# vsahni3/cross-attention-ViT

Hardware: AMD Instinct MI355X
Metric: 3D patch-tokens/sec fwd+bwd, 2-modality 128^3 p16 ViT (higher is better)
Workload: dtype bf16; 1 GPU; configs[1]: ModelCross d=768 H=12 mlp=3072 2x2 blocks, 2 modalities, 128^3 volume, 16^3 patches (N=513), dropout 0; per_gpu_batch=126, global_batch=126, seq_len=513, parallelism=dp1, step=zero-grad + weight bf16 cast + fwd + loss + bwd, optimizer_step=excluded, launch=eager (one launch per kernel)

## Files before the change

cross-attention-vit_amd/csrc/gemm.hip:

```cpp
#include "xvit_common.h"

#include <atomic>
#include <algorithm>
#include <string>

namespace xvit {

struct GemmParams {
  const bf16* A = nullptr; const bf16* B = nullptr; void* C = nullptr; const float* bias = nullptr; const float* res = nullptr; bf16* aux = nullptr;
  int64_t lda = 0, ldb = 0, ldc = 0, ldr = 0, ldaux = 0;
  int64_t sA = 0, sB = 0, sC = 0, sBias = 0, sR = 0, sAux = 0;
  int M = 0, N = 0, K = 0, k_per_split = 0, split_k = 1, ntm = 0, ntn = 0;
  int c_f32 = 0, act = XVIT_ACT_NONE, accumulate = 0;
  int res_row_mod = 0, res_row_off = 0, seg_rows = 0, seg_skip = 0, row_off = 0;
  float* slab = nullptr;
  float* colsum = nullptr;
  float drop_p = 0.f, drop_inv = 1.f; uint64_t drop_seed = 0;
  const uint64_t* drop_epoch = nullptr;
  int aux_deriv = 0;
  int narrow_epi = 0;
  int ncg = 1;
  int res_in_body = 0;
  struct PatchGather {
    int mode = 0;
    int dp, hp, wp;
    int Dn, Wn;
    int Sy, Sz;
    int pcount, ntok, cls;
    int nb;
    int64_t sBt, sMd;
    uint32_t vol_bytes;
    uint32_t m_pcount, m_dn, m_wn, m_nb;
    uint32_t m_ntok;
  } g;
};

constexpr uint32_t GATHER_OOB = 0x80000000u;
constexpr uint32_t OOB = 0xFFFFFFF0u;
typedef __attribute__((__vector_size__(2 * sizeof(unsigned)))) unsigned u32x2_t;
typedef __attribute__((__vector_size__(4 * sizeof(unsigned)))) unsigned u32x4_t;
__device__ __forceinline__ uint32_t gather_elem_off(const GemmParams::PatchGather& g, int e) {
  const int hw = g.hp * g.wp, p1 = e / hw, r = e - p1 * hw, p2 = r / g.wp, p3 = r - p2 * g.wp;
  return (uint32_t)(p1 * g.Sz + p2 * g.Sy + p3);
}
__device__ __forceinline__ uint32_t gather_patch_origin(const GemmParams::PatchGather& g, int q) {
  const int d = q % g.Dn, t = q / g.Dn, w = t % g.Wn, h = t / g.Wn;
  return (uint32_t)(d * g.dp * g.Sz + h * g.hp * g.Sy + w * g.wp);
}
__device__ __forceinline__ uint32_t gather_sample_origin(const GemmParams::PatchGather& g, int s) {
  const int mod = s / g.nb, b = s - mod * g.nb;
  return (uint32_t)(b * g.sBt + mod * g.sMd);
}

__device__ __forceinline__ uint32_t fast_div(uint32_t n, uint32_t d, uint32_t m, uint32_t& rem) {
  uint32_t q = __umulhi(n, m);
  rem = n - q * d;
  if (rem >= d) { ++q; rem -= d; }
  return q;
}
struct GatherTok { uint32_t row, vol; bool ok; };
__device__ __forceinline__ GatherTok gather_token(const GemmParams::PatchGather& g, uint32_t T, uint32_t total) {
  GatherTok o;
  o.ok = T < total;
  uint32_t q, b, d, w;
  const uint32_t smp = fast_div(o.ok ? T : 0u, (uint32_t)g.pcount, g.m_pcount, q);
  const uint32_t mod = fast_div(smp, (uint32_t)g.nb, g.m_nb, b);
  const uint32_t t = fast_div(q, (uint32_t)g.Dn, g.m_dn, d);
  const uint32_t h = fast_div(t, (uint32_t)g.Wn, g.m_wn, w);
  o.row = smp * (uint32_t)g.ntok + (uint32_t)g.cls + q;
  o.vol = (uint32_t)(b * g.sBt + mod * g.sMd) + d * (uint32_t)(g.dp * g.Sz) + h * (uint32_t)(g.hp * g.Sy) + w * (uint32_t)g.wp;
  return o;
}

constexpr int ACT_GELU_D = 3;
constexpr int ACT_MULAUX = 4;

template <int ACT>
__device__ __forceinline__ void act4(f32x4& v, f32x4& d, const bf16x4 z) {
  if (ACT == XVIT_ACT_GELU || ACT == ACT_GELU_D) {
#pragma unroll
    for (int c = 0; c < 4; ++c) { float a_, d_; gelu_and_grad(v[c], a_, d_); v[c] = a_; d[c] = d_; }
  } else if (ACT == XVIT_ACT_DGELU) {
#pragma unroll
    for (int c = 0; c < 4; ++c) v[c] *= dgelu_f(bf2f(z[c]));
  } else if (ACT == ACT_MULAUX) {
#pragma unroll
    for (int c = 0; c < 4; ++c) v[c] *= bf2f(z[c]);
  }
}
__device__ __forceinline__ void dropout4(const GemmParams& p, f32x4& v, uint64_t idx) {
  const uint32_t thr = (uint32_t)(p.drop_p * kTwo24);
  const uint64_t seed = drop_seed_at(p.drop_seed, p.drop_epoch);
#pragma unroll
  for (int c = 0; c < 4; ++c) v[c] = draw24(seed, idx + c) >= thr ? v[c] * p.drop_inv : 0.f;
}
template <int GROUP>
__device__ __forceinline__ void colsum_flush(float* dst, f32x4 cs, bool col_ok) {
#pragma unroll
  for (int c = 0; c < 4; ++c) {
    float t = cs[c];
#pragma unroll
    for (int o = GROUP; o < 64; o <<= 1) t += __shfl_xor(t, o);
    cs[c] = t;
  }
  if ((threadIdx.x & 63) < GROUP && col_ok) {
#pragma unroll
    for (int c = 0; c < 4; ++c) unsafeAtomicAdd(dst + c, cs[c]);
  }
}

template <int ACT, bool DROP = false>
__device__ __forceinline__ f32x4 epilogue_apply(const GemmParams& p, f32x4 v, int row, int col, int64_t cb, const float* bias, const float* res,
                                                bf16* aux) {
  if (bias) v += *(const f32x4*)(bias + col);
  if (ACT == XVIT_ACT_GELU) {
    f32x4 d;
    const f32x4 zv = v;
    act4<XVIT_ACT_GELU>(v, d, bf16x4{});
    if (aux) {
      const f32x4 s = p.aux_deriv ? d : zv;
      *(bf16x4*)(aux + (int64_t)row * p.ldaux + col) = to_bf16x4(s);
    }
  } else if (ACT == XVIT_ACT_DGELU) {
    const bf16x4 z = *(const bf16x4*)(aux + (int64_t)row * p.ldaux + col);
    f32x4 d;
    if (p.aux_deriv) act4<ACT_MULAUX>(v, d, z);
    else act4<XVIT_ACT_DGELU>(v, d, z);
  }
  if (DROP) dropout4(p, v, (uint64_t)(cb / (p.sC ? p.sC : 1)) * ((uint64_t)p.M * p.N) + (uint64_t)row * p.N + col);
  if (res) {
    const int rr = p.res_row_mod > 0 ? p.res_row_off + (row % p.res_row_mod) : row;
    v += *(const f32x4*)(res + (int64_t)rr * p.ldr + col);
  }
  const int64_t orow = p.seg_rows > 0 ? (int64_t)row + (row / p.seg_rows) * p.seg_skip + p.row_off : row;
  if (p.c_f32) {
    float* dst = (float*)p.C + cb + orow * p.ldc + col;
    if (p.accumulate) v += *(const f32x4*)dst;
    *(f32x4*)dst = v;
  } else {
    *(bf16x4*)((bf16*)p.C + cb + orow * p.ldc + col) = to_bf16x4(v);
  }
  return v;
}
__device__ __forceinline__ f32x4 epilogue_apply_rt(const GemmParams& p, f32x4 v, int row, int col, int64_t cb, const float* bias, const float* res,
                                                   bf16* aux) {
  if (p.drop_p > 0.f) {
    if (p.act == XVIT_ACT_GELU) return epilogue_apply<XVIT_ACT_GELU, true>(p, v, row, col, cb, bias, res, aux);
    if (p.act == XVIT_ACT_DGELU) return epilogue_apply<XVIT_ACT_DGELU, true>(p, v, row, col, cb, bias, res, aux);
    return epilogue_apply<XVIT_ACT_NONE, true>(p, v, row, col, cb, bias, res, aux);
  }
  if (p.act == XVIT_ACT_GELU) return epilogue_apply<XVIT_ACT_GELU>(p, v, row, col, cb, bias, res, aux);
  if (p.act == XVIT_ACT_DGELU) return epilogue_apply<XVIT_ACT_DGELU>(p, v, row, col, cb, bias, res, aux);
  return epilogue_apply<XVIT_ACT_NONE>(p, v, row, col, cb, bias, res, aux);
}

constexpr int BM = 128, BN = 128, BK = 64;
constexpr int OPER_BYTES = BM * BK * 2;
constexpr int STAGE_BYTES = 2 * OPER_BYTES;
// ... 556 lines not shown
  const int64_t celt = p.c_f32 ? 4 : 2;
  e.rc = make_rsrc((const char*)p.C + batch * p.sC * celt, clamp_bytes(0x7FFFFFF0ll));
  e.has_aux = p.aux != nullptr; e.has_res = p.res != nullptr; e.to_slab = p.slab != nullptr;
  const bool has_bias = p.bias != nullptr;
  e.raux = make_rsrc(e.has_aux ? (const void*)(p.aux + batch * p.sAux) : (const void*)p.C, e.has_aux ? 0x7FFFFFF0u : 0u);
  e.rres = make_rsrc(e.has_res ? (const void*)(p.res + batch * p.sR) : (const void*)p.C, e.has_res ? 0x7FFFFFF0u : 0u);
  const __amdgpu_buffer_rsrc_t rbias = make_rsrc(has_bias ? (const void*)(p.bias + batch * p.sBias) : (const void*)p.C, has_bias ? (uint32_t)(p.N * 4) : 0u);
  e.rslab = make_rsrc(e.to_slab ? (const void*)(p.slab + ((int64_t)split * nbatch + batch) * (int64_t)p.M * p.N) : (const void*)p.C,
                      e.to_slab ? clamp_bytes((int64_t)p.M * p.N * 4) : 0u);
  const int wl = pin_lane(lane);
  uint32_t woff[8], roff[4];
  {
    const int r = wl & 15, g = wl >> 4, k = wl & 15, rr = wl >> 4;
#pragma unroll
    for (int j = 0; j < 4; ++j) woff[j] = woff[4 + j] = (uint32_t)(r * 256 + (((j * 4 + g) ^ r) << 4));
    if constexpr (PERM) {
#pragma unroll
      for (int half = 0; half < 2; ++half) {
        const int l32 = 16 * half + r, jj = l32 >> 3, ii = l32 & 7, rho = (ii & 3) * 8 + 2 * jj + (ii >> 2);
#pragma unroll
        for (int j = 0; j < 4; ++j) woff[half * 4 + j] = (uint32_t)(rho * 256 + (((j * 4 + g) ^ (rho & 15)) << 4));
      }
    }
#pragma unroll
    for (int q = 0; q < 4; ++q) roff[q] = (uint32_t)(rr * 256 + ((k ^ (q * 4 + rr)) << 4));
  }
  XVIT_LDS char* slice = smem + wave * EPI_WAVE_BYTES;
  e.col = (uint32_t)(col0 + (wl & 15) * 4);
  e.col_ok = e.col < (uint32_t)p.N;
  e.bias = __builtin_bit_cast(f32x4, __builtin_amdgcn_raw_buffer_load_b128(rbias, e.col * 4, 0, 0));
  e.drop_base = (uint64_t)batch * ((uint64_t)p.M * p.N);
  e.csum = f32x4{0.f, 0.f, 0.f, 0.f};
  e.colsum_dst = p.colsum ? p.colsum + batch * p.sBias + e.col : nullptr;
  e.row = (uint32_t)(row0 + (wl >> 4));
  {
    const bool rmap = p.res_row_mod > 0, smap = p.seg_rows > 0;
    e.rmod = rmap ? (uint32_t)p.res_row_mod : 0x7FFFFFFFu;
    e.smod = smap ? (uint32_t)p.seg_rows : 0x7FFFFFFFu;
    e.rrem = rmap ? e.row % e.rmod : e.row;
    e.srem = smap ? e.row % e.smod : e.row;
    const uint32_t rrow = rmap ? (uint32_t)p.res_row_off + e.rrem : e.row;
    const uint32_t orow = smap ? e.row + (e.row / e.smod) * (uint32_t)p.seg_skip + (uint32_t)p.row_off : e.row;
    const uint32_t ce = p.c_f32 ? 4u : 2u;
    e.c = orow * (uint32_t)p.ldc * ce + e.col * ce;
    e.aux = e.row * (uint32_t)p.ldaux * 2u + e.col * 2u;
    e.res = rrow * (uint32_t)p.ldr * 4u + e.col * 4u;
    e.slab = e.row * (uint32_t)p.N * 4u + e.col * 4u;
    e.c_step = 4u * (uint32_t)p.ldc * ce;
    e.aux_step = 4u * (uint32_t)p.ldaux * 2u;
    e.res_step = 4u * (uint32_t)p.ldr * 4u;
    e.slab_step = 4u * (uint32_t)p.N * 4u;
    e.c_gap = smap ? (uint32_t)p.seg_skip * (uint32_t)p.ldc * ce : 0u;
    e.res_wrap = rmap ? e.rmod * (uint32_t)p.ldr * 4u : 0u;
    if (rmap && e.rmod <= 4u) {
      if (e.rmod == 3u) { e.rrem *= 4u; e.rmod = 12u; e.res_step = (uint32_t)p.ldr * 4u; }
      else { e.rmod = 0x7FFFFFFFu; e.res_step = 0u; e.res_wrap = 0u; }
    }
    if (smap && e.smod <= 4u) {
      if (e.smod == 3u) { e.srem *= 4u; e.smod = 12u; e.c_step += e.c_gap; }
      else { e.c_step += (e.smod == 1u ? 4u : e.smod == 2u ? 2u : 1u) * e.c_gap; e.smod = 0x7FFFFFFFu; }
    }
  }
  const bool res_pf = RES_PF && e.has_res && !e.to_slab && !p.accumulate && p.act == XVIT_ACT_NONE && p.drop_p == 0.f && !p.res_in_body;
  if constexpr (PERM) {
    if (res_pf) big_epilogue<XVIT_ACT_NONE, false, true, true>(p, e, acc, slice, woff, roff);
    else big_epilogue<XVIT_ACT_NONE, false, true>(p, e, acc, slice, woff, roff);
    return;
  }
  if constexpr (RES_PF) {
    if (res_pf) {
      big_epilogue<XVIT_ACT_NONE, false, false, true>(p, e, acc, slice, woff, roff);
      return;
    }
  }
  if (p.drop_p > 0.f) {
    if (p.act == XVIT_ACT_GELU) big_epilogue<XVIT_ACT_GELU, true>(p, e, acc, slice, woff, roff);
    else if (p.act == XVIT_ACT_DGELU) big_epilogue<XVIT_ACT_DGELU, true>(p, e, acc, slice, woff, roff);
    else big_epilogue<XVIT_ACT_NONE, true>(p, e, acc, slice, woff, roff);
  } else if (p.act == XVIT_ACT_GELU) big_epilogue<XVIT_ACT_GELU, false>(p, e, acc, slice, woff, roff);
  else if (p.act == XVIT_ACT_DGELU) big_epilogue<XVIT_ACT_DGELU, false>(p, e, acc, slice, woff, roff);
  else big_epilogue<XVIT_ACT_NONE, false>(p, e, acc, slice, woff, roff);
}

struct ScatterEpi {
  char* vol;
  uint32_t eoff;
  bool col_ok;
  uint32_t row;
};

__device__ __forceinline__ void scatter_body(const GemmParams& p, ScatterEpi& e, f32x4 v0, f32x4 v1) {
  const GemmParams::PatchGather& g = p.g;
  const uint32_t row = e.row;
  e.row += 8;
  if (!e.col_ok || row >= (uint32_t)p.M) return;
  uint32_t n, b, d, w;
  const uint32_t smp = fast_div(row, (uint32_t)g.ntok, g.m_ntok, n);
  if (n < (uint32_t)g.cls) return;
  const uint32_t t = fast_div(n - (uint32_t)g.cls, (uint32_t)g.Dn, g.m_dn, d);
  const uint32_t h = fast_div(t, (uint32_t)g.Wn, g.m_wn, w);
  const uint32_t mod = fast_div(smp, (uint32_t)g.nb, g.m_nb, b);
  const uint32_t off = b * (uint32_t)g.sBt + mod * (uint32_t)g.sMd + d * (uint32_t)(g.dp * g.Sz) + h * (uint32_t)(g.hp * g.Sy) + w * (uint32_t)g.wp + e.eoff;
  if (p.c_f32) {
    f32x4* dst = (f32x4*)((float*)e.vol + off);
    dst[0] = v0;
    dst[1] = v1;
  } else {
    *(u32x4_t*)((bf16*)e.vol + off) = pack_bf16x8(v0, v1);
  }
}

__device__ __forceinline__ void scatter_epilogue(const GemmParams& p, const f32x4 (&acc)[8][4], XVIT_LDS char* smem, int wave, int lane, int row0, int col0) {
  const int wl = pin_lane(lane);
  Transpose8 t;
  t.init(wl);
  ScatterEpi e;
  e.vol = (char*)p.C;
  const uint32_t col = (uint32_t)(col0 + (wl & 7) * 8);
  e.col_ok = col < (uint32_t)p.N;
  e.eoff = e.col_ok ? gather_elem_off(p.g, (int)col) : 0u;
  e.row = (uint32_t)(row0 + (wl >> 3));
  struct NoLoads {} none;
  transpose8_regions<0>(t, acc, smem + wave * EPI_WAVE_BYTES, none, [](NoLoads&) {}, [&](f32x4 v0, f32x4 v1, const NoLoads&, int) { scatter_body(p, e, v0, v1); });
}

#ifdef XVIT_GEMM_CLOCK_PROBE
__device__ long long xvit_dbg_clk[2 * 4096];
__device__ long long xvit_dbg_seg[3 * 4096];
struct ClockProbe {
  long long c0, w0, t[3] = {0, 0, 0};
  __device__ ClockProbe() : c0(clock64()), w0(wall_clock64()) {}
  __device__ void mark(int i) { if (t[i] == 0) t[i] = clock64(); }
  __device__ ~ClockProbe() {
    if (threadIdx.x == 0 && blockIdx.z == 0 && blockIdx.x < 4096) {
      xvit_dbg_clk[2 * blockIdx.x] = clock64() - c0; xvit_dbg_clk[2 * blockIdx.x + 1] = wall_clock64() - w0;
      for (int i = 0; i < 3; ++i) xvit_dbg_seg[3 * blockIdx.x + i] = t[i] - c0;
    }
  }
};
#define XVIT_PROBE_MARK(i) clock_probe.mark(i)
#else
#define XVIT_PROBE_MARK(i)
#endif
template <bool A_KS, bool B_KS, int WIDE_ACT, int GATHER = 0>
__global__ __launch_bounds__(512, 2) void gemm_big_kernel(const GemmParams p) {
  extern __shared__ __attribute__((aligned(16))) char smem_raw[];
  XVIT_LDS char* smem = (XVIT_LDS char*)smem_raw;
#ifdef XVIT_GEMM_CLOCK_PROBE
  ClockProbe clock_probe;
#endif
  const int tid = threadIdx.x, lane = tid & 63, wave = uniform(tid >> 6);
  const int wr = wave >> 2, wc = wave & 3;

  const int nblk = gridDim.x;
  const int logical = xcd_logical(blockIdx.x + nblk * blockIdx.z, nblk * gridDim.z);
  const int zz = logical / nblk, tile = logical - zz * nblk;
  const int grp = min(tile / (p.ntm * p.ncg), (p.ntn - 1) / p.ncg);
  const int rem = tile - grp * p.ntm * p.ncg;
  const int gw = min(p.ncg, p.ntn - grp * p.ncg);
  const int tm = rem / gw, tn = grp * p.ncg + (rem - tm * gw);
  const int m0 = tm * TBM, n0 = tn * TBN;
  const int batch = zz / p.split_k, split = zz - batch * p.split_k;
  const int k_begin = split * p.k_per_split;
  const int k_end = min(p.K, k_begin + p.k_per_split);
  const int nk = (k_end - k_begin + BK - 1) / BK;

// ... 1 lines not shown
  TileLoader<B_KS, TBN> lb;
  {
    const bf16* Ab = p.A + batch * p.sA;
    if constexpr (GATHER == 1) la.init_gather_rows(p.g, Ab, m0, p.M, wave, lane);
    else if constexpr (GATHER == 2 || GATHER == 3) {
      const int64_t rows = (int64_t)(p.K / p.g.pcount) * p.g.ntok;
      la.init(OperandTile{Ab + m0, ((rows - 1) * p.lda + (p.M - m0)) * 2}, p.lda, wave, lane, GATHER == 2 ? &p.g : nullptr);
    } else la.init(operand_tile<A_KS>(Ab, p.lda, m0, p.M, k_begin, k_end), p.lda, wave, lane);
    const bf16* Bb = p.B + batch * p.sB;
    if constexpr (GATHER == 2 || GATHER == 3) lb.init_gather_ks(p.g, Bb, n0, p.N, wave, lane);
    else lb.init(operand_tile<B_KS>(Bb, p.ldb, n0, p.N, k_begin, k_end), p.ldb, wave, lane);
  }
  const int ktg0 = k_begin / BK;
  uint32_t fix_a[4], fix_b[4];
  if constexpr (GATHER == 3) {
    la.init_token_fixed(p.g, m0, p.M, false, fix_a, wave, lane);
    lb.init_token_fixed(p.g, n0, p.N, true, fix_b, wave, lane);
  }
  auto step_off = [&](int kt, uint32_t& oa, uint32_t& ob) {
    if constexpr (GATHER == 1) { oa = gather_soff_rows(p.g, ktg0 + kt); ob = (uint32_t)kt * lb.kstep; }
    else if constexpr (GATHER == 2) { GatherStep o; o = gather_soff_wgrad(p.g, ktg0 + kt, p.lda); oa = o.a; ob = o.b; }
    else if constexpr (GATHER == 3) {
      la.place_tokens(p.g, ktg0 + kt, (uint32_t)p.K, p.lda, false, fix_a, wave, lane);
      lb.place_tokens(p.g, ktg0 + kt, (uint32_t)p.K, 0, true, fix_b, wave, lane);
      oa = ob = 0u;
    }
    else { oa = (uint32_t)kt * la.kstep; ob = (uint32_t)kt * lb.kstep; }
  };
  TileFrag<A_KS, TBM, 8> fa;
  TileFrag<B_KS, TBN, 4> fb;
  fa.init(wr * 8, lane);
  fb.init(wc * 4, lane);

  f32x4 acc[8][4];
#pragma unroll
  for (int i = 0; i < 8; ++i)
#pragma unroll
    for (int j = 0; j < 4; ++j) acc[i][j] = f32x4{0.f, 0.f, 0.f, 0.f};

  const __amdgpu_buffer_rsrc_t null_rsrc = make_rsrc(p.A, 0u);
  if (nk > 0) {
    uint32_t oa, ob;
    step_off(0, oa, ob);
    la.issue_at(smem, wave, oa);
    lb.issue_at(smem + T_OPER, wave, ob);
  }
  for (int kt = 0; kt < nk; ++kt) {
    asm volatile("s_waitcnt vmcnt(0)" ::: "memory");
    __syncthreads();
    XVIT_PROBE_MARK(0);
    const bool more = kt + 1 < nk;
    uint32_t soff_a, soff_b;
    step_off(kt + 1, soff_a, soff_b);
    XVIT_LDS char* nxt = smem + ((kt + 1) & 1) * T_STAGE;
    const XVIT_LDS char* sa = smem + (kt & 1) * T_STAGE;
    const XVIT_LDS char* sb = sa + T_OPER;
#ifndef XVIT_DEBUG_NO_MMA
    big_tile_mma<A_KS, B_KS>(sa, sb, fa, fb, acc, la, lb, more ? la.rsrc : null_rsrc, more ? lb.rsrc : null_rsrc, nxt, wave, soff_a, soff_b);
#endif
  }
  XVIT_PROBE_MARK(1);

  asm volatile("s_waitcnt vmcnt(0)" ::: "memory");
  __syncthreads();
  if constexpr (GATHER == 4) scatter_epilogue(p, acc, smem, wave, lane, m0 + wr * 128, n0 + wc * 64);
  else if constexpr (WIDE_ACT >= 0) wave_tile_epilogue_wide<WIDE_ACT>(p, acc, smem, wave, lane, m0 + wr * 128, n0 + wc * 64, batch);
  else wave_tile_epilogue<GATHER == 1, GATHER <= 1>(p, acc, smem, wave, lane, m0 + wr * 128, n0 + wc * 64, batch, split);
  XVIT_PROBE_MARK(2);
}

__device__ __forceinline__ const GemmParams& reload_params() {
  auto q = __builtin_amdgcn_kernarg_segment_ptr();
  asm volatile("" : "+s"(q));
  return *(const GemmParams*)q;
}

template <bool B_KS, int WIDE_ACT>
__global__ __launch_bounds__(512, 2) void gemm_big_loop_kernel(const GemmParams p) {
  extern __shared__ __attribute__((aligned(16))) char smem_raw[];
  XVIT_LDS char* smem = (XVIT_LDS char*)smem_raw;
#ifdef XVIT_GEMM_CLOCK_PROBE
  ClockProbe clock_probe;
#endif
  static_assert(WIDE_ACT >= 0, "the tile loop exists behind the wide epilogues only");
  constexpr int EPI_STORES = 16;
  const int tid = threadIdx.x, lane = tid & 63, wave = uniform(tid >> 6);
  const int wr = wave >> 2, wc = wave & 3;
  auto tile_origin = [](const GemmParams& q, int slot, int& m0, int& n0) {
    const int tile = xcd_logical(slot, q.ntm * q.ntn);
    const int grp = min(tile / (q.ntm * q.ncg), (q.ntn - 1) / q.ncg);
    const int rem = tile - grp * q.ntm * q.ncg;
    const int gw = min(q.ncg, q.ntn - grp * q.ncg);
    const int tm = rem / gw, tn = grp * q.ncg + (rem - tm * gw);
    m0 = tm * TBM; n0 = tn * TBN;
  };
  auto tile_rsrc = [](const GemmParams& q, int m0, int n0, __amdgpu_buffer_rsrc_t& ra, __amdgpu_buffer_rsrc_t& rb) {
    const OperandTile ta = operand_tile<false>(q.A, q.lda, m0, q.M, 0, q.K), tb = operand_tile<B_KS>(q.B, q.ldb, n0, q.N, 0, q.K);
    ra = make_rsrc(ta.base, clamp_bytes(ta.bytes));
    rb = make_rsrc(tb.base, clamp_bytes(tb.bytes));
  };
  TileLoader<false, TBM> la;
  TileLoader<B_KS, TBN> lb;
  la.init(OperandTile{p.A, 0}, p.lda, wave, lane);
  lb.init(OperandTile{p.B, 0}, p.ldb, wave, lane);
  TileFrag<false, TBM, 8> fa;
  TileFrag<B_KS, TBN, 4> fb;
  fa.init(wr * 8, lane);
  fb.init(wc * 4, lane);

  int slot = blockIdx.x;
  int stage = 0;
  int m0, n0;
  tile_origin(p, slot, m0, n0);
  tile_rsrc(p, m0, n0, la.rsrc, lb.rsrc);
  la.issue_at(smem, wave, 0u);
  lb.issue_at(smem + T_OPER, wave, 0u);
  for (;;) {
    const bool first = slot == (int)blockIdx.x;
    const int nk = (reload_params().K + BK - 1) / BK;
    f32x4 acc[8][4];
#pragma unroll
    for (int i = 0; i < 8; ++i)
#pragma unroll
      for (int j = 0; j < 4; ++j) acc[i][j] = f32x4{0.f, 0.f, 0.f, 0.f};
    for (int kt = 0; kt + 1 < nk; ++kt) {
      if (kt == 0 && !first) wait_vmcnt<EPI_STORES>();
      else wait_vmcnt<0>();
      __syncthreads();
      XVIT_PROBE_MARK(0);
      XVIT_LDS char* nxt = smem + ((stage + kt + 1) & 1) * T_STAGE;
      const XVIT_LDS char* sa = smem + ((stage + kt) & 1) * T_STAGE;
      big_tile_mma<false, B_KS>(sa, sa + T_OPER, fa, fb, acc, la, lb, la.rsrc, lb.rsrc, nxt, wave, (uint32_t)(kt + 1) * la.kstep, (uint32_t)(kt + 1) * lb.kstep);
    }
    bool more;
    int nm0 = 0, nn0 = 0;
    __amdgpu_buffer_rsrc_t ra = make_rsrc(nullptr, 0u), rb = ra;
    {
      const GemmParams& q = reload_params();
      more = slot + (int)gridDim.x < q.ntm * q.ntn;
      if (more) {
        tile_origin(q, slot + (int)gridDim.x, nm0, nn0);
        tile_rsrc(q, nm0, nn0, ra, rb);
      }
    }
    if (nk == 1 && !first) wait_vmcnt<EPI_STORES>();
    else wait_vmcnt<0>();
    __syncthreads();
    XVIT_PROBE_MARK(0);
    {
      const XVIT_LDS char* sa = smem + ((stage + nk - 1) & 1) * T_STAGE;
      big_tile_mma<false, B_KS>(sa, sa + T_OPER, fa, fb, acc, la, lb, ra, rb, smem + ((stage + nk) & 1) * T_STAGE, wave, 0u, 0u);
    }
    XVIT_PROBE_MARK(1);
    if (!more) wait_vmcnt<0>();
    __syncthreads();
    {
      const GemmParams& q = reload_params();
      const int te = pin_lane(tid), we = uniform(te >> 6);
      XVIT_LDS char* slices = smem + ((stage + nk - 1) & 1) * T_STAGE;
      wave_tile_epilogue_wide<WIDE_ACT, 32>(q, acc, slices, we, te & 63, m0 + (we >> 2) * 128, n0 + (we & 3) * 64, 0);
    }
    XVIT_PROBE_MARK(2);
    if (!more) break;
    la.rsrc = ra; lb.rsrc = rb;
    m0 = nm0; n0 = nn0;
    slot += (int)gridDim.x;
    stage = (stage + nk) & 1;
  }
}

__global__ void splitk_epilogue_kernel(const GemmParams p, int nbatch) {
  const int nv = p.N >> 2;
  const int64_t per = (int64_t)p.M * nv, total = per * nbatch;
  for (int64_t i = (int64_t)blockIdx.x * blockDim.x + threadIdx.x; i < total; i += (int64_t)gridDim.x * blockDim.x) {
    const int b = (int)(i / per);
    const int64_t r = i - (int64_t)b * per;
    const int row = (int)(r / nv), col = (int)(r - (int64_t)row * nv) * 4;
    f32x4 v = {0.f, 0.f, 0.f, 0.f};
    for (int s = 0; s < p.split_k; ++s) v += *(const f32x4*)(p.slab + (((int64_t)s * nbatch + b) * p.M + row) * p.N + col);
    const f32x4 o = epilogue_apply_rt(p, v, row, col, b * p.sC, p.bias ? p.bias + b * p.sBias : nullptr, p.res ? p.res + b * p.sR : nullptr,
                                      p.aux ? p.aux + b * p.sAux : nullptr);
    if (p.colsum) {
#pragma unroll
      for (int e = 0; e < 4; ++e) unsafeAtomicAdd(p.colsum + b * p.sBias + col + e, o[e]);
    }
  }
}

}

using namespace xvit;

static bool aligned16(const void* p) { return (reinterpret_cast<uintptr_t>(p) & 15) == 0; }

static std::atomic<int> g_gemm_tile{0};
static std::atomic<int> g_gemm_epi{0};
static std::atomic<int> g_gemm_res_pf{0};
static std::atomic<int> g_gemm_group{0};

static std::atomic<int> g_gemm_persist{0};

static int cu_count() {
  static const int n = [] {
    int dev = 0, v = 0;
    if (hipGetDevice(&dev) != hipSuccess || hipDeviceGetAttribute(&v, hipDeviceAttributeMultiprocessorCount, dev) != hipSuccess) v = 0;
    return v;
  }();
  return n;
}

static int loop_workgroups(const xvit_gemm_args* a, const GemmParams& p, int grid_z) {
  const int opt = g_gemm_persist.load(std::memory_order_relaxed);
  if (opt == 1 || a->layout == XVIT_GEMM_TN || grid_z != 1) return 0;
  const int tiles = p.ntm * p.ntn;
  if (opt >= 2) return std::min(tiles, opt);
  const int cus = cu_count();
  if (cus <= 0 || tiles < 2 * cus) return 0;
  if (p.K > 768 || (p.act != XVIT_ACT_NONE && !p.aux_deriv)) return 0;
  return cus;
}

static bool use_big_tile(const xvit_gemm_args* a) {
  if (a->M < 256 || a->N < 256 || g_gemm_tile.load(std::memory_order_relaxed) == 1) return false;
  if (g_gemm_tile.load(std::memory_order_relaxed) == 2) return true;
  const int64_t big_blocks = (int64_t)((a->M + 255) / 256) * ((a->N + 255) / 256) * a->batch * (a->split_k > 0 ? a->split_k : 1);
  return big_blocks > 128;
}

static int k_per_split(int K, int split_k) {
  const int ktiles = (K + BK - 1) / BK;
  return ((ktiles + split_k - 1) / split_k) * BK;
}

static void set_tile_grid(GemmParams& p, int tile, int layout, bool grouped = true) {
  p.ntm = (p.M + tile - 1) / tile; p.ntn = (p.N + tile - 1) / tile;
  p.ncg = p.ntn;
  if (grouped) {
    const int forced = g_gemm_group.load(std::memory_order_relaxed);
    p.ncg = forced > 0 ? std::min(forced, p.ntn) : (layout == XVIT_GEMM_NT && p.ntn >= 6 ? 3 : p.ntn);
  }
}

template <bool A_KS, bool B_KS, int WIDE_ACT, int GATHER = 0>
static void launch_big(const GemmParams& p, int grid_z, hipStream_t s) {
  launch_lds<gemm_big_kernel<A_KS, B_KS, WIDE_ACT, GATHER>, T_LDS, 512>(dim3(p.ntm * p.ntn, 1, grid_z), s, p);
}
template <bool B_KS, int WIDE_ACT>
static void launch_loop(const GemmParams& p, int wgs, hipStream_t s) {
  launch_lds<gemm_big_loop_kernel<B_KS, WIDE_ACT>, T_LDS, 512>(dim3(wgs, 1, 1), s, p);
}
template <bool A_KS, bool B_KS>
static void launch_small(const GemmParams& p, int grid_z, hipStream_t s) {
  launch_lds<gemm_kernel<A_KS, B_KS>, GEMM_LDS, 256>(dim3(p.ntm * p.ntn, 1, grid_z), s, p);
}
static void launch_splitk_reduce(const GemmParams& p, int nbatch, hipStream_t s) {
  const int64_t work = (int64_t)nbatch * p.M * (p.N / 4);
  const int g = (int)((work + 255) / 256 > 4096 ? 4096 : (work + 255) / 256);
  hipLaunchKernelGGL(splitk_epilogue_kernel, dim3(g), dim3(256), 0, s, p, nbatch);
}

extern "C" int xvit_set_option(const char* name, int value) {
  XVIT_REQUIRE(name != nullptr, "xvit_set_option: null name");
  const std::string n(name);
  if (n == "gemm_tile") { XVIT_REQUIRE(value >= 0 && value <= 2, "xvit_set_option: gemm_tile must be 0 (auto), 1 (128x128 only) or 2 (256x256 whenever M, N >= 256)"); g_gemm_tile = value; return 0; }
  if (n == "gemm_group") { XVIT_REQUIRE(value >= 0 && value <= 4096, "xvit_set_option: gemm_group must be in [0, 4096]"); g_gemm_group = value; return 0; }
  if (n == "gemm_epilogue") { XVIT_REQUIRE(value == 0 || value == 1, "xvit_set_option: gemm_epilogue must be 0 (auto) or 1 (narrow)"); g_gemm_epi = value; return 0; }
  if (n == "gemm_persistent") { XVIT_REQUIRE(value >= 0 && value <= 4096, "xvit_set_option: gemm_persistent must be 0 (auto), 1 (one workgroup per tile) or 2..4096 (the tile loop on at most that many workgroups)"); g_gemm_persist = value; return 0; }
  if (n == "gemm_res_prefetch") { XVIT_REQUIRE(value == 0 || value == 1, "xvit_set_option: gemm_res_prefetch must be 0 (one region ahead) or 1 (in the body)"); g_gemm_res_pf = value; return 0; }
  if (n == "attn_peel") { XVIT_REQUIRE(value >= 0 && value <= 2, "xvit_set_option: attn_peel must be 0 (token 0 stays on the tile grid), 1 (auto: large grids) or 2 (whenever N = 64 m + 1)"); set_attn_peel(value); return 0; }
  set_error("xvit_set_option: unknown option '%s'", name);
  return XVIT_ERR_ARG;
}

extern "C" int64_t xvit_gemm_workspace_bytes(const xvit_gemm_args* a) {
  if (!a || a->split_k <= 1) return 0;
  return (int64_t)a->split_k * a->batch * a->M * a->N * (int64_t)sizeof(float);
}

extern "C" int xvit_gemm(const xvit_gemm_args* a, xvit_stream_t stream) {
  XVIT_REQUIRE(a != nullptr, "xvit_gemm: null args");
  XVIT_REQUIRE(a->layout >= 0 && a->layout <= 2, "xvit_gemm: bad layout %d", a->layout);
  XVIT_REQUIRE(a->M > 0 && a->N > 0 && a->K > 0 && a->batch > 0, "xvit_gemm: M,N,K,batch must be > 0 (got %d,%d,%d,%d)", a->M, a->N, a->K, a->batch);
  XVIT_REQUIRE(a->A && a->B && a->C, "xvit_gemm: null A/B/C");
  const bool a_ks = a->layout == XVIT_GEMM_TN, b_ks = a->layout != XVIT_GEMM_NT;
  XVIT_REQUIRE(a_ks || a->K % 64 == 0, "xvit_gemm: K=%d must be a multiple of 64 when A is k-contiguous", a->K);
  XVIT_REQUIRE(b_ks || a->K % 64 == 0, "xvit_gemm: K=%d must be a multiple of 64 when B is k-contiguous", a->K);
  XVIT_REQUIRE(a->N % 4 == 0, "xvit_gemm: N=%d must be a multiple of 4 (use xvit_small_linear_*)", a->N);
  XVIT_REQUIRE(a->lda % 8 == 0 && a->ldb % 8 == 0 && a->stride_a % 8 == 0 && a->stride_b % 8 == 0, "xvit_gemm: lda/ldb/strides must be multiples of 8 elements");
  XVIT_REQUIRE(aligned16(a->A) && aligned16(a->B) && aligned16(a->C), "xvit_gemm: A/B/C must be 16-byte aligned");
  XVIT_REQUIRE(a->ldc % 4 == 0 && a->stride_c % 4 == 0, "xvit_gemm: ldc/stride_c must be multiples of 4");
  XVIT_REQUIRE(a->lda >= (a_ks ? a->M : a->K) && a->ldb >= (b_ks ? a->N : a->K) && a->ldc >= a->N, "xvit_gemm: leading dimension smaller than the row length");
  const int64_t a_rows = a_ks ? a->K : a->M, b_rows = b_ks ? a->K : a->N;
  XVIT_REQUIRE(a_rows * a->lda * 2 < (1ll << 31) && b_rows * a->ldb * 2 < (1ll << 31), "xvit_gemm: an operand matrix exceeds 2 GiB (unsupported addressing range)");
  XVIT_REQUIRE(a->split_k >= 1, "xvit_gemm: split_k must be >= 1");
  {
    const int64_t out_rows = a->out_seg_rows > 0 ? (int64_t)a->M + (a->M / a->out_seg_rows + 1) * a->out_seg_skip + a->out_row_off : a->M;
    XVIT_REQUIRE(out_rows * a->ldc * 4 < (1ll << 31) && (!a->aux || (int64_t)a->M * a->ldaux * 2 < (1ll << 31)) &&
                     (!a->residual || (int64_t)a->M * a->ldr * 4 < (1ll << 31)),
                 "xvit_gemm: C / aux / residual of one batch exceed 2 GiB (unsupported addressing range)");
  }
  XVIT_REQUIRE(!(a->accumulate && a->c_dtype != XVIT_F32), "xvit_gemm: accumulate needs fp32 C");
  XVIT_REQUIRE(a->act != XVIT_ACT_DGELU || a->aux, "xvit_gemm: ACT_DGELU needs aux (pre-activation)");
  XVIT_REQUIRE(a->aux_mode == 0 || a->aux_mode == 1, "xvit_gemm: aux_mode must be 0 (aux = pre-activation) or 1 (aux = GELU')");
  if (a->aux) XVIT_REQUIRE(a->ldaux % 4 == 0 && a->ldaux >= a->N && (reinterpret_cast<uintptr_t>(a->aux) & 7) == 0, "xvit_gemm: bad aux layout");
  if (a->residual) XVIT_REQUIRE(a->ldr % 4 == 0 && a->ldr >= a->N && aligned16(a->residual), "xvit_gemm: bad residual layout");
  if (a->bias) XVIT_REQUIRE(aligned16(a->bias) && a->stride_bias % 4 == 0, "xvit_gemm: bias must be 16-byte aligned");
  XVIT_REQUIRE((int64_t)a->batch * a->split_k <= 65535, "xvit_gemm: batch*split_k too large");
  const bool big = use_big_tile(a);
  const int64_t ws_need = xvit_gemm_workspace_bytes(a);
  if (ws_need > 0)
    XVIT_REQUIRE(a->workspace && a->workspace_bytes >= ws_need && aligned16(a->workspace), "xvit_gemm: split_k=%d needs %lld bytes of 16-byte aligned workspace (got %lld)",
                 a->split_k, (long long)ws_need, (long long)a->workspace_bytes);

  GemmParams p;
  p.A = (const bf16*)a->A; p.B = (const bf16*)a->B; p.C = a->C; p.bias = a->bias; p.res = a->residual; p.aux = (bf16*)a->aux;
  p.lda = a->lda; p.ldb = a->ldb; p.ldc = a->ldc; p.ldr = a->ldr; p.ldaux = a->ldaux;
  p.sA = a->stride_a; p.sB = a->stride_b; p.sC = a->stride_c; p.sBias = a->stride_bias; p.sR = a->stride_r; p.sAux = a->stride_aux;
  p.M = a->M; p.N = a->N; p.K = a->K; p.split_k = a->split_k;
  p.k_per_split = k_per_split(a->K, a->split_k);
  p.c_f32 = a->c_dtype == XVIT_F32; p.act = a->act; p.accumulate = a->accumulate;
  p.res_row_mod = a->res_row_mod; p.res_row_off = a->res_row_off;
  p.seg_rows = a->out_seg_rows; p.seg_skip = a->out_seg_skip; p.row_off = a->out_row_off;
  p.slab = ws_need > 0 ? (float*)a->workspace : nullptr;
  p.colsum = a->colsum;
  XVIT_REQUIRE(a->dropout_p >= 0.f && a->dropout_p < 1.f, "xvit_gemm: dropout_p must be in [0, 1)");
  p.drop_p = a->dropout_p; p.drop_inv = 1.0f / (1.0f - a->dropout_p); p.drop_seed = a->dropout_seed;
  p.drop_epoch = a->dropout_p > 0.f ? drop_epoch_ptr() : nullptr;
  p.narrow_epi = g_gemm_epi.load(std::memory_order_relaxed);
  p.res_in_body = g_gemm_res_pf.load(std::memory_order_relaxed);
  p.aux_deriv = a->aux_mode;
  hipStream_t s = (hipStream_t)stream;
  const int gz = a->batch * a->split_k;

  if (big) {
    set_tile_grid(p, TBM, a->layout);
    const bool wide = !p.c_f32 && !p.slab && !p.res && p.seg_rows == 0 && !p.narrow_epi && p.drop_p == 0.f && a->layout != XVIT_GEMM_TN &&
                      ((p.N | (int)p.ldc | (int)p.ldaux) & 7) == 0 && (a->layout == XVIT_GEMM_NT ? p.act != XVIT_ACT_DGELU : p.act != XVIT_ACT_GELU);
    const int lw = wide ? loop_workgroups(a, p, gz) : 0;
    if (wide && a->layout == XVIT_GEMM_NT && p.act == XVIT_ACT_NONE) lw ? launch_loop<false, XVIT_ACT_NONE>(p, lw, s) : launch_big<false, false, XVIT_ACT_NONE>(p, gz, s);
    else if (wide && a->layout == XVIT_GEMM_NT && p.aux_deriv) lw ? launch_loop<false, ACT_GELU_D>(p, lw, s) : launch_big<false, false, ACT_GELU_D>(p, gz, s);
    else if (wide && a->layout == XVIT_GEMM_NT) lw ? launch_loop<false, XVIT_ACT_GELU>(p, lw, s) : launch_big<false, false, XVIT_ACT_GELU>(p, gz, s);
    else if (wide && p.act == XVIT_ACT_NONE) lw ? launch_loop<true, XVIT_ACT_NONE>(p, lw, s) : launch_big<false, true, XVIT_ACT_NONE>(p, gz, s);
    else if (wide && p.aux_deriv) lw ? launch_loop<true, ACT_MULAUX>(p, lw, s) : launch_big<false, true, ACT_MULAUX>(p, gz, s);
    else if (wide) lw ? launch_loop<true, XVIT_ACT_DGELU>(p, lw, s) : launch_big<false, true, XVIT_ACT_DGELU>(p, gz, s);
    else if (a->layout == XVIT_GEMM_NT) launch_big<false, false, -1>(p, gz, s);
    else if (a->layout == XVIT_GEMM_NN) launch_big<false, true, -1>(p, gz, s);
    else launch_big<true, true, -1>(p, gz, s);
  } else {
    set_tile_grid(p, BM, a->layout, false);
    switch (a->layout) {
      case XVIT_GEMM_NT: launch_small<false, false>(p, gz, s); break;
      case XVIT_GEMM_NN: launch_small<false, true>(p, gz, s); break;
      default: launch_small<true, true>(p, gz, s); break;
    }
  }
  if (p.slab) launch_splitk_reduce(p, a->batch, s);
  return check_launch("xvit_gemm");
}

static int64_t pe_rows(const xvit_patch_geom* g) {
  return (int64_t)g->M * g->B * (g->cls_rows + (int64_t)(g->D / g->dp) * (g->H / g->hp) * (g->W / g->wp));
}

static bool pe_geom_ok(const xvit_patch_geom* g) {
  if (!g || g->B <= 0 || g->M <= 0 || g->dp <= 0 || g->hp <= 0 || g->wp <= 0 || (g->cls_rows != 0 && g->cls_rows != 1)) return false;
  return !(g->D % g->dp || g->H % g->hp || g->W % g->wp);
}

extern "C" int xvit_patch_embed_supported(const xvit_patch_geom* g, int d) {
  if (!pe_geom_ok(g)) return 0;
  const int Dn = g->D / g->dp, Hn = g->H / g->hp, Wn = g->W / g->wp;
  const int64_t pd = (int64_t)g->dp * g->hp * g->wp, pcount = (int64_t)Dn * Hn * Wn;
  if (g->wp % 8 || 64 % g->wp || (g->hp * g->wp) % 64) return 0;
  if (pd % 256 || d % 256 || d < 256) return 0;
  const int64_t rows = pe_rows(g);
  if (rows < 2048) return 0;
  if ((int64_t)g->B * g->M * g->D * g->H * g->W * 2 >= (1ll << 31)) return 0;
  if (rows * d * 4 >= (1ll << 31) || pcount > (1 << 24)) return 0;
  return 1;
}

static bool pe_aligned(const xvit_patch_geom* g) {
  const int Dn = g->D / g->dp, Wn = g->W / g->wp;
  return 64 % Dn == 0 && (Dn * Wn) % 64 == 0;
}

static void pe_fill(GemmParams& p, const xvit_patch_geom* g, int mode) {
  p.g.mode = mode;
  p.g.dp = g->dp; p.g.hp = g->hp; p.g.wp = g->wp;
  p.g.Dn = g->D / g->dp; p.g.Wn = g->W / g->wp;
  p.g.Sy = g->W; p.g.Sz = g->H * g->W;
  p.g.pcount = (g->D / g->dp) * (g->H / g->hp) * (g->W / g->wp);
  p.g.cls = g->cls_rows; p.g.ntok = p.g.cls + p.g.pcount;
  p.g.nb = g->B;
  p.g.sMd = (int64_t)g->D * g->H * g->W; p.g.sBt = p.g.sMd * g->M;
  p.g.vol_bytes = (uint32_t)((int64_t)g->B * g->M * g->D * g->H * g->W * 2);
  auto magic = [](int d) { return d <= 1 ? 0xFFFFFFFFu : (uint32_t)((1ull << 32) / (uint64_t)d); };
  p.g.m_pcount = magic(p.g.pcount); p.g.m_dn = magic(p.g.Dn); p.g.m_wn = magic(p.g.Wn); p.g.m_nb = magic(p.g.nb); p.g.m_ntok = magic(p.g.ntok);
}

static void pe_defaults(GemmParams& p) {
  p.c_f32 = 1; p.narrow_epi = 1;
}

extern "C" int xvit_patch_embed_fwd(const void* img, const xvit_patch_geom* g, const void* W, int64_t ldw, const float* bias, const float* pos, int64_t ldpos,
                                    float* x, int64_t ldx, int d, xvit_stream_t stream) {
  XVIT_REQUIRE(img && g && W && x, "xvit_patch_embed_fwd: null pointer");
  XVIT_REQUIRE(xvit_patch_embed_supported(g, d) == 1, "xvit_patch_embed_fwd: geometry not supported by the fused kernel (xvit_patch_embed_supported)");
  const int64_t pd = (int64_t)g->dp * g->hp * g->wp;
  XVIT_REQUIRE(ldw >= pd && ldw % 8 == 0 && ldx >= d && ldx % 4 == 0 && (!pos || (ldpos >= d && ldpos % 4 == 0)), "xvit_patch_embed_fwd: bad leading dimension");
  XVIT_REQUIRE(aligned16(img) && aligned16(W) && aligned16(x) && (!bias || aligned16(bias)) && (!pos || aligned16(pos)), "xvit_patch_embed_fwd: pointers must be 16-byte aligned");
  GemmParams p;
  pe_defaults(p);
  pe_fill(p, g, 1);
  p.A = (const bf16*)img; p.B = (const bf16*)W; p.C = x; p.bias = bias; p.res = pos;
  p.ldb = ldw; p.ldc = ldx; p.ldr = ldpos;
  p.M = (int)pe_rows(g); p.N = d; p.K = (int)pd;
  p.k_per_split = p.K;
  p.res_in_body = g_gemm_res_pf.load(std::memory_order_relaxed);
  if (pos) { p.res_row_mod = p.g.ntok; p.res_row_off = 0; }
  set_tile_grid(p, TBM, XVIT_GEMM_NT, false);
  launch_big<false, false, -1, 1>(p, 1, (hipStream_t)stream);
  return check_launch("xvit_patch_embed_fwd");
}

static int pe_wgrad_split(const xvit_patch_geom* g, int d) {
  const int64_t pd = (int64_t)g->dp * g->hp * g->wp;
// ... 83 lines not shown
```

Before: 3.828 million patch-tokens/s.

## Route f32 residual GEMMs through persistent tile loop with staggered epilogue phases

Adds a persistent tile-loop variant for NT GEMMs that write f32 output with a residual add and bias. Its epilogue prefetches the next residual region while storing the current one. Half of the workgroups, in alternating groups of eight, sleep for a short modeled delay at start so that epilogue store bursts and K-loop compute fall out of phase across CUs. The cost is extra idle time at kernel start and a heuristic delay model built from hardcoded per-step timings.

```diff
diff --git a/cross-attention-vit_amd/csrc/gemm.hip b/cross-attention-vit_amd/csrc/gemm.hip
--- a/cross-attention-vit_amd/csrc/gemm.hip
+++ b/cross-attention-vit_amd/csrc/gemm.hip
@@ -21,6 +21,7 @@
   int narrow_epi = 0;
   int ncg = 1;
   int res_in_body = 0;
+  int phase_wgs = 0, phase_ticks = 0;
   struct PatchGather {
     int mode = 0;
     int dp, hp, wp;
@@ -74,6 +75,7 @@
 
 constexpr int ACT_GELU_D = 3;
 constexpr int ACT_MULAUX = 4;
+constexpr int ACT_RES32 = 5;
 
 template <int ACT>
 __device__ __forceinline__ void act4(f32x4& v, f32x4& d, const bf16x4 z) {
@@ -796,6 +798,85 @@
   else big_epilogue<XVIT_ACT_NONE, false>(p, e, acc, slice, woff, roff);
 }
 
+struct Res32Epi {
+  __amdgpu_buffer_rsrc_t rc, rres;
+  bool col_ok;
+  f32x4 bias;
+  uint32_t row, c;
+  uint32_t lrow, lres;
+  uint32_t c_step, res_step;
+};
+struct Res32Loads { u32x4_t res[4]; };
+
+__device__ __forceinline__ void res32_issue(int M, Res32Epi& e, Res32Loads& L) {
+#pragma unroll
+  for (int b = 0; b < 4; ++b) {
+    const bool ok = e.col_ok && e.lrow < (uint32_t)M;
+    L.res[b] = __builtin_amdgcn_raw_buffer_load_b128(e.rres, ok ? e.lres : OOB, 0, XVIT_EPI_RES_AUX);
+    e.lrow += 4; e.lres += e.res_step;
+  }
+}
+
+template <int R, int PASS>
+__device__ __forceinline__ void res32_regions(int M, Res32Epi& e, Res32Loads& cur, const f32x4 (&acc)[8][4], XVIT_LDS char* slice, const uint32_t (&woff)[4],
+                                              const uint32_t (&roff)[4]) {
+  constexpr int RPP = PASS / 16;
+  if constexpr (R % RPP == 0) {
+#pragma unroll
+    for (int i = 0; i < RPP; ++i)
+#pragma unroll
+      for (int j = 0; j < 4; ++j) *(XVIT_LDS f32x4*)(slice + i * 4096 + woff[j]) = acc[R + i][j];
+  }
+  Res32Loads nxt;
+  if constexpr (R < 7) res32_issue(M, e, nxt);
+#pragma unroll
+  for (int b = 0; b < 4; ++b) {
+    const int it = (R % RPP) * 4 + b;
+    f32x4 v = *(const XVIT_LDS f32x4*)(slice + it * 1024 + roff[it & 3]);
+    const bool ok = e.col_ok && e.row < (uint32_t)M;
+    v += e.bias;
+    v += __builtin_bit_cast(f32x4, cur.res[b]);
+    __builtin_amdgcn_raw_buffer_store_b128(__builtin_bit_cast(u32x4_t, v), e.rc, ok ? e.c : OOB, 0, XVIT_EPI_STORE_AUX);
+    e.row += 4; e.c += e.c_step;
+  }
+  __builtin_amdgcn_sched_barrier(0);
+  if constexpr (R < 7) res32_regions<R + 1, PASS>(M, e, nxt, acc, slice, woff, roff);
+}
+
+template <int PASS = 64>
+__device__ __forceinline__ void wave_tile_epilogue_res32(const GemmParams& p, const f32x4 (&acc)[8][4], XVIT_LDS char* smem, int wave, int lane, int row0, int col0,
+                                                         int batch) {
+  Res32Epi e;
+  e.rc = make_rsrc((const char*)p.C + batch * p.sC * 4, clamp_bytes(0x7FFFFFF0ll));
+  e.rres = make_rsrc(p.res + batch * p.sR, 0x7FFFFFF0u);
+  const bool has_bias = p.bias != nullptr;
+  const __amdgpu_buffer_rsrc_t rbias = make_rsrc(has_bias ? (const void*)(p.bias + batch * p.sBias) : (const void*)p.C, has_bias ? (uint32_t)(p.N * 4) : 0u);
+  const int wl = pin_lane(lane);
+  uint32_t woff[4], roff[4];
+  const int r = wl & 15, g = wl >> 4;
+#pragma unroll
+  for (int j = 0; j < 4; ++j) woff[j] = (uint32_t)(r * 256 + (((j * 4 + g) ^ r) << 4));
+#pragma unroll
+  for (int q = 0; q < 4; ++q) roff[q] = (uint32_t)(g * 256 + ((r ^ (q * 4 + g)) << 4));
+  const uint32_t col = (uint32_t)(col0 + r * 4);
+  e.col_ok = col < (uint32_t)p.N;
+  e.bias = __builtin_bit_cast(f32x4, __builtin_amdgcn_raw_buffer_load_b128(rbias, col * 4, 0, 0));
+  e.row = e.lrow = (uint32_t)(row0 + g);
+  e.c = e.row * (uint32_t)p.ldc * 4u + col * 4u;
+  e.lres = e.row * (uint32_t)p.ldr * 4u + col * 4u;
+  e.c_step = 16u * (uint32_t)p.ldc;
+  e.res_step = 16u * (uint32_t)p.ldr;
+  Res32Loads first;
+  res32_issue(p.M, e, first);
+  res32_regions<0, PASS>(p.M, e, first, acc, smem + wave * (PASS * 256), woff, roff);
+}
+
+__device__ __forceinline__ void phase_wait(const GemmParams& p, int dispatch_index) {
+  if (p.phase_ticks <= 0 || dispatch_index >= p.phase_wgs || ((dispatch_index >> 3) & 1) == 0) return;
+  const uint64_t t0 = wall_clock64();
+  for (int i = 0; i < 512 && wall_clock64() - t0 < (uint64_t)p.phase_ticks; ++i) __builtin_amdgcn_s_sleep(8);
+}
+
 struct ScatterEpi {
   char* vol;
   uint32_t eoff;
@@ -963,8 +1044,9 @@
 #ifdef XVIT_GEMM_CLOCK_PROBE
   ClockProbe clock_probe;
 #endif
-  static_assert(WIDE_ACT >= 0, "the tile loop exists behind the wide epilogues only");
-  constexpr int EPI_STORES = 16;
+  static_assert(WIDE_ACT >= 0, "the tile loop exists behind the compile-time epilogues only");
+  constexpr int EPI_STORES = WIDE_ACT == ACT_RES32 ? 32 : 16;
+  if constexpr (WIDE_ACT == ACT_RES32) phase_wait(p, (int)blockIdx.x);
   const int tid = threadIdx.x, lane = tid & 63, wave = uniform(tid >> 6);
   const int wr = wave >> 2, wc = wave & 3;
   auto tile_origin = [](const GemmParams& q, int slot, int& m0, int& n0) {
@@ -1039,7 +1121,8 @@
       const GemmParams& q = reload_params();
       const int te = pin_lane(tid), we = uniform(te >> 6);
       XVIT_LDS char* slices = smem + ((stage + nk - 1) & 1) * T_STAGE;
-      wave_tile_epilogue_wide<WIDE_ACT, 32>(q, acc, slices, we, te & 63, m0 + (we >> 2) * 128, n0 + (we & 3) * 64, 0);
+      if constexpr (WIDE_ACT == ACT_RES32) wave_tile_epilogue_res32<32>(q, acc, slices, we, te & 63, m0 + (we >> 2) * 128, n0 + (we & 3) * 64, 0);
+      else wave_tile_epilogue_wide<WIDE_ACT, 32>(q, acc, slices, we, te & 63, m0 + (we >> 2) * 128, n0 + (we & 3) * 64, 0);
     }
     XVIT_PROBE_MARK(2);
     if (!more) break;
@@ -1081,6 +1164,10 @@
 
 static std::atomic<int> g_gemm_persist{0};
 
+static std::atomic<int> g_gemm_epi_phase{0};
+static std::atomic<int> g_gemm_epi_phase_us{0};
+constexpr int PHASE_CAP_US = 40;
+
 static int cu_count() {
   static const int n = [] {
     int dev = 0, v = 0;
@@ -1090,15 +1177,30 @@
   return n;
 }
 
-static int loop_workgroups(const xvit_gemm_args* a, const GemmParams& p, int grid_z) {
+static int loop_workgroups(const xvit_gemm_args* a, const GemmParams& p, int grid_z, bool res32 = false) {
   const int opt = g_gemm_persist.load(std::memory_order_relaxed);
   if (opt == 1 || a->layout == XVIT_GEMM_TN || grid_z != 1) return 0;
   const int tiles = p.ntm * p.ntn;
   if (opt >= 2) return std::min(tiles, opt);
   const int cus = cu_count();
   if (cus <= 0 || tiles < 2 * cus) return 0;
+  if (res32) return p.K <= 768 || p.K >= 3072 ? cus : 0;
   if (p.K > 768 || (p.act != XVIT_ACT_NONE && !p.aux_deriv)) return 0;
   return cus;
+}
+
+static int phase_ticks(const GemmParams& p, int grid_z) {
+  const int opt = g_gemm_epi_phase.load(std::memory_order_relaxed);
+  const int cus = cu_count();
+  if (opt == 1 || grid_z != 1 || cus <= 0) return 0;
+  const bool tuned = p.K <= 768;
+  if (opt == 0 && !(tuned && p.ntm * p.ntn >= 2 * cus)) return 0;
+  constexpr double EPI_US = 23.9, KSTEP_US = 1.4, PROLOGUE_US = 2.4, TUNED_US = 10.0;
+  const double kloop = KSTEP_US * ((p.K + BK - 1) / BK);
+  const double rule = tuned ? TUNED_US : kloop > EPI_US ? EPI_US : 0.5 * (PROLOGUE_US + kloop + EPI_US);
+  const int forced = g_gemm_epi_phase_us.load(std::memory_order_relaxed);
+  const double us = std::min<double>(PHASE_CAP_US, forced > 0 ? forced : rule);
+  return (int)(us * 100.0);
 }
 
 static bool use_big_tile(const xvit_gemm_args* a) {
@@ -1147,6 +1249,8 @@
   if (n == "gemm_group") { XVIT_REQUIRE(value >= 0 && value <= 4096, "xvit_set_option: gemm_group must be in [0, 4096]"); g_gemm_group = value; return 0; }
   if (n == "gemm_epilogue") { XVIT_REQUIRE(value == 0 || value == 1, "xvit_set_option: gemm_epilogue must be 0 (auto) or 1 (narrow)"); g_gemm_epi = value; return 0; }
   if (n == "gemm_persistent") { XVIT_REQUIRE(value >= 0 && value <= 4096, "xvit_set_option: gemm_persistent must be 0 (auto), 1 (one workgroup per tile) or 2..4096 (the tile loop on at most that many workgroups)"); g_gemm_persist = value; return 0; }
+  if (n == "gemm_epi_phase") { XVIT_REQUIRE(value >= 0 && value <= 2, "xvit_set_option: gemm_epi_phase must be 0 (auto), 1 (off) or 2 (phase groups wherever they exist)"); g_gemm_epi_phase = value; return 0; }
+  if (n == "gemm_epi_phase_us") { XVIT_REQUIRE(value >= 0 && value <= PHASE_CAP_US, "xvit_set_option: gemm_epi_phase_us must be 0 (the rule's delay) or 1..%d us", PHASE_CAP_US); g_gemm_epi_phase_us = value; return 0; }
   if (n == "gemm_res_prefetch") { XVIT_REQUIRE(value == 0 || value == 1, "xvit_set_option: gemm_res_prefetch must be 0 (one region ahead) or 1 (in the body)"); g_gemm_res_pf = value; return 0; }
   if (n == "attn_peel") { XVIT_REQUIRE(value >= 0 && value <= 2, "xvit_set_option: attn_peel must be 0 (token 0 stays on the tile grid), 1 (auto: large grids) or 2 (whenever N = 64 m + 1)"); set_attn_peel(value); return 0; }
   set_error("xvit_set_option: unknown option '%s'", name);
@@ -1217,13 +1321,21 @@
     set_tile_grid(p, TBM, a->layout);
     const bool wide = !p.c_f32 && !p.slab && !p.res && p.seg_rows == 0 && !p.narrow_epi && p.drop_p == 0.f && a->layout != XVIT_GEMM_TN &&
                       ((p.N | (int)p.ldc | (int)p.ldaux) & 7) == 0 && (a->layout == XVIT_GEMM_NT ? p.act != XVIT_ACT_DGELU : p.act != XVIT_ACT_GELU);
-    const int lw = wide ? loop_workgroups(a, p, gz) : 0;
+    const bool res32_ok = a->layout == XVIT_GEMM_NT && p.c_f32 && p.res && !p.slab && !p.accumulate && p.act == XVIT_ACT_NONE && p.drop_p == 0.f && !p.colsum &&
+                       p.res_row_mod == 0 && p.seg_rows == 0 && !p.narrow_epi && !p.res_in_body;
+    const int lw = wide ? loop_workgroups(a, p, gz) : res32_ok ? loop_workgroups(a, p, gz, true) : 0;
+    const bool res32 = res32_ok && lw > 0;
+    if (res32) {
+      p.phase_wgs = lw;
+      p.phase_ticks = phase_ticks(p, gz);
+    }
     if (wide && a->layout == XVIT_GEMM_NT && p.act == XVIT_ACT_NONE) lw ? launch_loop<false, XVIT_ACT_NONE>(p, lw, s) : launch_big<false, false, XVIT_ACT_NONE>(p, gz, s);
     else if (wide && a->layout == XVIT_GEMM_NT && p.aux_deriv) lw ? launch_loop<false, ACT_GELU_D>(p, lw, s) : launch_big<false, false, ACT_GELU_D>(p, gz, s);
     else if (wide && a->layout == XVIT_GEMM_NT) lw ? launch_loop<false, XVIT_ACT_GELU>(p, lw, s) : launch_big<false, false, XVIT_ACT_GELU>(p, gz, s);
     else if (wide && p.act == XVIT_ACT_NONE) lw ? launch_loop<true, XVIT_ACT_NONE>(p, lw, s) : launch_big<false, true, XVIT_ACT_NONE>(p, gz, s);
     else if (wide && p.aux_deriv) lw ? launch_loop<true, ACT_MULAUX>(p, lw, s) : launch_big<false, true, ACT_MULAUX>(p, gz, s);
     else if (wide) lw ? launch_loop<true, XVIT_ACT_DGELU>(p, lw, s) : launch_big<false, true, XVIT_ACT_DGELU>(p, gz, s);
+    else if (res32) launch_loop<false, ACT_RES32>(p, lw, s);
     else if (a->layout == XVIT_GEMM_NT) launch_big<false, false, -1>(p, gz, s);
     else if (a->layout == XVIT_GEMM_NN) launch_big<false, true, -1>(p, gz, s);
     else launch_big<true, true, -1>(p, gz, s);
```

After: 3.835 million patch-tokens/s, median of 6. Within noise of the previous version (+0.2%).
